# scverse/scanpy

Hardware: AMD Instinct MI355X
Metric: cells/sec through pca+neighbors+leiden, 1M x 2k CSR (higher is better)
Workload: dtype bf16x3

## Files before the change

### scanpy_amd/csrc/leiden.hip

```cpp
#include "common.h"
#include "scan.h"

#include <algorithm>
#include <cmath>
#include <cstdlib>
#include <ctime>
#include <type_traits>

namespace scamd {

enum LdStat : int {
  ST_ITERATIONS = 0, ST_LAUNCHES, ST_ROUND_TRIPS, ST_POLISH_FULL_SWEEPS, ST_POLISH_ROUNDS, ST_POLISH_MOVES,
  ST_POLISH_SKIPPED_PROVEN, ST_LEVELS_FIRST_ITER, ST_LM_SWEEPS, ST_LM_SWEEP_MB, ST_POLISH_SPLITS, ST_ENDED_BY_ITER_CAP,
  ST_POLISH_ROUND_CAP, ST_ITER_CAP, ST_UNUSED_14, ST_DEVICE_FILLS, ST_LEVELS_REUSED, ST_QUIET_REUSE_ITERS,
  ST_OVERFLOW_VERTICES, ST_HUB_VERTICES, LD_NSTATS
};
static_assert(LD_NSTATS == 20 && ST_UNUSED_14 == 14, "the slot numbers are part of the C ABI (scamd_leiden_last_stats)");
struct LdStatName {
  int slot;
  const char* key;
};
static const LdStatName LD_STAT_NAMES[] = {
    {ST_ITERATIONS, "iterations"},
    {ST_LAUNCHES, "launches"},
    {ST_ROUND_TRIPS, "host_round_trips"},
    {ST_POLISH_FULL_SWEEPS, "polish_full_sweeps"},
    {ST_POLISH_ROUNDS, "polish_rounds"},
    {ST_POLISH_MOVES, "polish_moves"},
    {ST_POLISH_SKIPPED_PROVEN, "polish_skipped_proven"},
    {ST_LEVELS_FIRST_ITER, "levels_first_iteration"},
    {ST_LM_SWEEPS, "lm_sweeps"},
    {ST_LM_SWEEP_MB, "lm_sweep_algorithmic_MB"},
    {ST_POLISH_SPLITS, "polish_splits"},
    {ST_ENDED_BY_ITER_CAP, "ended_by_iteration_cap"},
    {ST_POLISH_ROUND_CAP, "polish_ended_by_round_cap"},
    {ST_ITER_CAP, "iteration_cap"},
    {ST_DEVICE_FILLS, "device_fills"},
    {ST_LEVELS_REUSED, "levels_reused"},
    {ST_QUIET_REUSE_ITERS, "quiet_reuse_iterations"},
    {ST_OVERFLOW_VERTICES, "overflow_pass_vertices"},
    {ST_HUB_VERTICES, "hub_pass_vertices"},
};
constexpr int G16_SLOTS = 128;
constexpr int G16_MAX = G16_SLOTS * 3 / 4;
static thread_local int g_ld_stats[LD_NSTATS] = {0};
static thread_local double g_ld_sweep_bytes = 0.0;
#undef SCAMD_LAUNCH_CHECK
#define SCAMD_LAUNCH_CHECK()                \
  do {                                      \
    ++g_ld_stats[ST_LAUNCHES];              \
    SCAMD_HIP_CHECK(hipGetLastError());     \
  } while (0)
#define LD_FETCH(dst, src, bytes, stream)                                          \
  do {                                                                             \
    const int rc_fetch_ = host_readback().fetch((dst), (src), (bytes), (stream)); \
    if (rc_fetch_ != SCAMD_OK) return rc_fetch_;                                   \
  } while (0)
#define LD_SYNC(stream)                                       \
  do {                                                        \
    ++g_ld_stats[ST_ROUND_TRIPS];                             \
    const int rc_sync_ = host_readback().sync(stream);        \
    if (rc_sync_ != SCAMD_OK) return rc_sync_;                \
  } while (0)

constexpr double WSCALE = 4294967296.0;
constexpr int MAX_LM_SWEEPS = 96;
constexpr int LM_DIR_AFTER = 32;
constexpr int MAX_CLASSES = 32;
constexpr int DEF_CLASSES = 8;
constexpr int CTR_STRIDE = 16;
constexpr int CTR_JOINED = 0, CTR_N_MID = 8, CTR_N_BLK = 9, CTR_N_GIANT = 10;
constexpr int PH_PER_PHASE = 8;
constexpr int PH_MOVED = 0, PH_BLOCKED = 1;
constexpr int PH_CC_CHANGED = 2, PH_CC_COMPONENTS = 3, PH_CC_COMMUNITIES = 4;
constexpr int PH_AGG_PART_SLOTS = 2, PH_AGG_PARTS = 3, PH_AGG_MID = 4, PH_AGG_BIG = 5, PH_AGG_SPLIT = 6;
constexpr int PHASE_ERR = 7;
constexpr int PH_MAX_DEG = 8;
constexpr int PH_SMALL_INFO = 12, SM_INFO_LEVELS = 0, SM_INFO_MOVES = 1, SM_INFO_MERGES = 2, SM_INFO_NODES = 3;
constexpr int CTR_AREA = MAX_CLASSES + CTR_STRIDE * MAX_CLASSES;
constexpr int MAX_LEVELS = 64;
constexpr int MAX_OUTER_ITERS = 32;

__host__ __device__ __forceinline__ unsigned int hash32(unsigned int x) {
  x ^= x >> 16;
  x *= 0x7feb352dU;
  x ^= x >> 15;
  x *= 0x846ca68bU;
  x ^= x >> 16;
  return x;
}
__device__ __forceinline__ unsigned int prio(int c, unsigned int seed) { return hash32((unsigned int)c ^ seed); }

__device__ __forceinline__ long long readlane_i64(long long v, int l) {
  int lo = __builtin_amdgcn_readlane((int)(v & 0xffffffffll), l);
  int hi = __builtin_amdgcn_readlane((int)(v >> 32), l);
  return ((long long)hi << 32) | (unsigned int)lo;
}

__global__ void ld_quantize_kernel(const float* __restrict__ w, int64_t nnz, long long* __restrict__ wq) {
  int64_t e = (int64_t)blockIdx.x * blockDim.x + threadIdx.x;
  if (e < nnz) {
    double v = (double)w[e];
    wq[e] = (v > 0.0) ? (long long)llrint(v * WSCALE) : 0ll;
  }
}

__global__ void ld_strength_kernel(const int64_t* __restrict__ indptr, const long long* __restrict__ wq, int n,
                                   long long* __restrict__ k) {
  const int lane = threadIdx.x & 63;
  const int v = blockIdx.x * (blockDim.x >> 6) + (threadIdx.x >> 6);
  if (v >= n) return;
  long long s = 0;
  for (int64_t e = indptr[v] + lane; e < indptr[v + 1]; e += 64) s += wq[e];
#pragma unroll
  for (int o = 32; o > 0; o >>= 1) s += __shfl_xor(s, o);
  if (lane == 0) k[v] = s;
}

__global__ __launch_bounds__(256) void ld_sum_kernel(const long long* __restrict__ a, int n,
                                                     unsigned long long* __restrict__ total) {
  long long s = 0;
  for (int i = blockIdx.x * blockDim.x + threadIdx.x; i < n; i += gridDim.x * blockDim.x) s += a[i];
#pragma unroll
  for (int o = 32; o > 0; o >>= 1) s += __shfl_xor(s, o);
  if ((threadIdx.x & 63) == 0 && s != 0) atomicAdd(total, (unsigned long long)s);
}

__global__ __launch_bounds__(1024) void ld_degstats_kernel(const int64_t* __restrict__ indptr, int n, int* __restrict__ out) {
  __shared__ int sh;
  if (threadIdx.x == 0) sh = 0;
  __syncthreads();
  int v = blockIdx.x * blockDim.x + threadIdx.x;
  int d = (v < n) ? (int)(indptr[v + 1] - indptr[v]) : 0;
#pragma unroll
  for (int o = 32; o > 0; o >>= 1) d = max(d, __shfl_xor(d, o));
  if ((threadIdx.x & 63) == 0 && d > 0) atomicMax(&sh, d);
  __syncthreads();
  if (threadIdx.x == 0 && sh > 0) atomicMax(out, sh);
}

__global__ void ld_iota_kernel(int* __restrict__ a, int n) {
  int i = blockIdx.x * blockDim.x + threadIdx.x;
  if (i < n) a[i] = i;
}

constexpr double NODE_WEIGHT_SCALE = 65536.0;
__global__ void ld_nodeweight_quantize_kernel(const float* __restrict__ w, int n, long long* __restrict__ k, int* __restrict__ err) {
  const int v = blockIdx.x * blockDim.x + threadIdx.x;
  if (v >= n) return;
  const float x = w[v];
  if (!(x >= 0.f) || !(x <= 1.0e6f)) {
    atomicOr(err, 1);
    k[v] = 0ll;
    return;
  }
  k[v] = llrint((double)x * NODE_WEIGHT_SCALE);
// ... 1538 lines not shown
        const int64_t p = u0 + wbase + __popcll(m & ((1ull << lane) - 1ull));
        s_col[p] = key;
        s_w[p] = (long long)vals[sl];
      }
    }
    __syncthreads();
    if (threadIdx.x == 0) rowcnt[c] = sh_cnt;
    __syncthreads();
  }
}

__global__ __launch_bounds__(256) void ld_agg_compact_kernel(int nn, const int64_t* __restrict__ moff,
                                                             const int64_t* __restrict__ eoff,
                                                             const int64_t* __restrict__ indptr_new,
                                                             const int* __restrict__ s_col,
                                                             const long long* __restrict__ s_w,
                                                             int* __restrict__ out_col, long long* __restrict__ out_w,
                                                             int* __restrict__ dstat) {
  const int lane = threadIdx.x & 63;
  const int c = blockIdx.x * 4 + (threadIdx.x >> 6);
  if (blockIdx.x == 0 && threadIdx.x == 0) dstat[0] = 0;
  if (c >= nn) return;
  const int64_t u0 = eoff[moff[c]];
  const int64_t p0 = indptr_new[c];
  const int cnt = (int)(indptr_new[c + 1] - p0);
  for (int i = lane; i < cnt; i += 64) {
    out_col[p0 + i] = s_col[u0 + i];
    out_w[p0 + i] = s_w[u0 + i];
  }
}

constexpr int SMALL_N = 1024;
constexpr int SMALL_NNZ = 65536;
constexpr int SM_WAVES = 8;
constexpr int SM_THREADS = SM_WAVES * 64;

struct SmallArgs {
  const int64_t* indptr;
  const int* indices;
  const long long* wq;
  const long long* k;
  int n;
  int* ix[2];
  long long* w[2];
  int first_dst;
  int* comm;
  double gg;
  double inv_beta;
  unsigned int seed;
  int iter;
  int lm_stop_permille;
  int seq_n;
  int* info;
};

struct SmallLds {
  unsigned long long acc[SM_WAVES][SMALL_N];
  unsigned short touched[SM_WAVES][SMALL_N];
  unsigned long long Ktot[SMALL_N];
  long long kk[SMALL_N];
  int ip[SMALL_N + 1];
  int comm[SMALL_N];
  int csize[SMALL_N];
  unsigned short order[SMALL_N];
  unsigned short tail_of[SMALL_N];
  unsigned char flag[SMALL_N];
  int ref[SMALL_N];
  int refsize[SMALL_N];
  union {
    struct {
      unsigned long long Kref[SMALL_N];
      unsigned long long Eref[SMALL_N];
      long long a_in[SMALL_N];
      int stamp[SMALL_N];
    } rf;
    struct {
      int cid[SMALL_N];
      int members[SMALL_N];
      int moff[SMALL_N + 1];
      int rep[SMALL_N];
      int rowptr[SMALL_N + 1];
    } ag;
  } u;
  int tcnt[SM_WAVES];
  int dec[SM_WAVES];
  int rset[SM_WAVES];
  int scan_w[SM_WAVES];
  int s_n_act, s_moved, s_merged, s_nn;
};
static_assert(sizeof(SmallLds) <= 160 * 1024, "SmallLds must fit the 160 KB of LDS");

__device__ __forceinline__ int small_scan(int* x, int n, int* scan_w) {
  const int t = threadIdx.x, lane = t & 63, wv = t >> 6;
  const int i0 = 2 * t, i1 = 2 * t + 1;
  const int a0 = i0 < n ? x[i0] : 0, a1 = i1 < n ? x[i1] : 0;
  int inc = a0 + a1;
#pragma unroll
  for (int o = 1; o < 64; o <<= 1) {
    const int y = __shfl_up(inc, o);
    if (lane >= o) inc += y;
  }
  if (lane == 63) scan_w[wv] = inc;
  __syncthreads();
  int off = 0, tot = 0;
  for (int i = 0; i < SM_WAVES; ++i) {
    const int s = scan_w[i];
    if (i < wv) off += s;
    tot += s;
  }
  const int ex = off + inc - (a0 + a1);
  if (i0 < n) x[i0] = ex;
  if (i1 < n) x[i1] = ex + a0;
  __syncthreads();
  return tot;
}

template <typename P>
__device__ __forceinline__ int small_compact(int n, P pred, unsigned short* order, int* scan_w) {
  const int t = threadIdx.x, lane = t & 63, wv = t >> 6;
  int base = 0;
  for (int v0 = 0; v0 < n; v0 += SM_THREADS) {
    const int v = v0 + t;
    const bool f = v < n && pred(v);
    const unsigned long long m = __ballot(f);
    if (lane == 0) scan_w[wv] = __popcll(m);
    __syncthreads();
    int off = 0, tot = 0;
    for (int i = 0; i < SM_WAVES; ++i) {
      const int s = scan_w[i];
      if (i < wv) off += s;
      tot += s;
    }
    if (f) order[base + off + __popcll(m & ((1ull << lane) - 1ull))] = (unsigned short)v;
    base += tot;
    __syncthreads();
  }
  return base;
}

constexpr int SMALL_SEQ_N = 16;
__global__ __launch_bounds__(SM_THREADS) void ld_small_levels_kernel(SmallArgs a) {
// ... 292 lines not shown
          for (int mi = L.u.ag.moff[c]; mi < L.u.ag.moff[c + 1]; ++mi) {
            const int v = L.u.ag.members[mi];
            for (int e = L.ip[v] + lane; e < L.ip[v + 1]; e += 64) {
              const long long w = wq[e];
              if (w != 0) {
                const int key = L.u.ag.cid[ix[e]];
                const unsigned long long old = atomicAdd(&acc[key], (unsigned long long)w);
                if (old == 0ull) touched[atomicAdd(&L.tcnt[wv], 1)] = (unsigned short)key;
              }
            }
          }
          const int tc = __hip_atomic_load(&L.tcnt[wv], __ATOMIC_RELAXED, __HIP_MEMORY_SCOPE_WORKGROUP);
          long long ksum = 0;
          const int p0 = pass ? L.u.ag.rowptr[c] : 0;
          for (int i = lane; i < tc; i += 64) {
            const int col = touched[i];
            const unsigned long long s = acc[col];
            acc[col] = 0ull;
            if (pass) {
              nix[p0 + i] = col;
              nw[p0 + i] = (long long)s;
              ksum += (long long)s;
            }
          }
          if (pass) {
#pragma unroll
            for (int o = 32; o > 0; o >>= 1) ksum += __shfl_xor(ksum, o);
            if (lane == 0) L.kk[c] = ksum;
          } else if (lane == 0) {
            L.u.ag.rep[c] = tc;
          }
        }
      }
      __syncthreads();
      if (pass == 0) {
        for (int c = t; c < nn; c += SM_THREADS) L.u.ag.rowptr[c] = L.u.ag.rep[c];
        __syncthreads();
        const int nnz_new = small_scan(L.u.ag.rowptr, nn, L.scan_w);
        if (t == 0) L.u.ag.rowptr[nn] = nnz_new;
        __syncthreads();
      }
    }
    for (int c = t; c <= nn; c += SM_THREADS) L.ip[c] = L.u.ag.rowptr[c];
    for (int c = t; c < nn; c += SM_THREADS) L.comm[c] = L.csize[c];
    __threadfence();
    __syncthreads();
    ix = nix;
    wq = nw;
    dst ^= 1;
    n = nn;
  }
  __syncthreads();
  for (int i = t; i < n_in; i += SM_THREADS) a.comm[i] = L.comm[L.tail_of[i]];
  if (t == 0) {
    a.info[SM_INFO_LEVELS] = levels;
    a.info[SM_INFO_MOVES] = tot_moves;
    a.info[SM_INFO_MERGES] = tot_merges;
    a.info[SM_INFO_NODES] = n;
  }
}

template <int G>
__global__ __launch_bounds__(256) void ld_internal_kernel(int n, const int64_t* __restrict__ indptr,
                                                          const int* __restrict__ indices,
                                                          const long long* __restrict__ wq, const int* __restrict__ comm,
                                                          unsigned long long* __restrict__ internal) {
  const int lane = threadIdx.x & 63, sub = threadIdx.x % G;
  long long s = 0;
  for (int v = blockIdx.x * (256 / G) + threadIdx.x / G; v < n; v += gridDim.x * (256 / G)) {
    const int a = comm[v];
    const int64_t beg = indptr[v], end = indptr[v + 1];
    for (int64_t e = beg + sub; e < end; e += 4 * G) {
      int u[4], cu[4];
      long long we[4];
#pragma unroll
      for (int t = 0; t < 4; ++t) {
        const int64_t ee = e + t * G;
        u[t] = ee < end ? indices[ee] : v;
        we[t] = ee < end ? wq[ee] : 0ll;
      }
#pragma unroll
      for (int t = 0; t < 4; ++t) cu[t] = comm[u[t]];
#pragma unroll
      for (int t = 0; t < 4; ++t)
        if (cu[t] == a) s += we[t];
    }
  }
#pragma unroll
  for (int o = 32; o > 0; o >>= 1) s += __shfl_xor(s, o);
  __shared__ long long sh_s[4];
  if (lane == 0) sh_s[threadIdx.x >> 6] = s;
  __syncthreads();
  if (threadIdx.x == 0) {
    const long long tot = sh_s[0] + sh_s[1] + sh_s[2] + sh_s[3];
    if (tot != 0) atomicAdd(internal, (unsigned long long)tot);
  }
}

constexpr int SUMSQ_BLOCKS = 256;
__device__ __forceinline__ double block_sum_1024(double s, double* sh) {
  sh[threadIdx.x] = s;
  __syncthreads();
  for (int o = 512; o > 0; o >>= 1) {
    if ((int)threadIdx.x < o) sh[threadIdx.x] += sh[threadIdx.x + o];
    __syncthreads();
  }
  return sh[0];
// ... 158 lines not shown
  b->scan_tmp = ws.take<int64_t>((size_t)scan_num_blocks(n) + 2);
  b->cid = ws.take<int>(N);
  b->rep = ws.take<int>(N);
  b->comm_tmp = ws.take<int>(N);
  b->node_of = ws.take<int>(N);
  b->memb = ws.take<int>(N);
  b->memb_work = ws.take<int>(N);
  b->agg_col = ws.take<int>(E);
  b->agg_w = ws.take<long long>(E);
  b->mcount = ws.take<int>(N);
  b->moff = ws.take<int64_t>(N + 1);
  b->eoff = ws.take<int64_t>(N + 1);
  b->members = ws.take<int>(N);
  b->mdeg = ws.take<int>(N);
  b->mid_list = ws.take<int>(N);
  b->big_list = ws.take<int>(N);
  {
    const size_t slots = 3 * E / (size_t)agg_split_chunk() + 16;
    b->pmoff = ws.take<int64_t>(slots);
    b->part_list = ws.take<int>(slots);
    b->part_cnt = ws.take<int>(slots);
  }
  b->rowcnt = ws.take<int>(N);
  b->cursor = ws.take<int>(N);
  b->counters = ws.take<int>(16);
  b->rcounters = ws.take<int>(2 * CTR_AREA);
  b->total = ws.take<unsigned long long>(4);
  b->dscratch = ws.take<double>(4 + SUMSQ_BLOCKS);
  b->ckeys = ws.take<unsigned long long>(N);
  b->cids = ws.take<int>(N);
  b->newlabel = ws.take<int>(N);
  b->minmember = ws.take<int>(N);
}

#define GRID1(n) dim3((unsigned)ceil_div((n), 256)), dim3(256)
#define GRIDW(n) dim3((unsigned)ceil_div((n), 4)), dim3(256)
#define GRIDK(n) dim3((unsigned)ceil_div((n), 1024)), dim3(1024)
constexpr int HUB_GRID = 512;
constexpr int AGG_MID_GRID = 768;
constexpr int LM_STOP_PERMILLE = 20;
constexpr int LM_STOP_PERMILLE_BIG = 40;
constexpr size_t HUB_LDS = (size_t)BHUB_SLOTS * 12;

struct Hierarchy {
  int depth = 0;
  int end_level = -1;
  int end_kind = 0;
};
struct IterHierarchy {
  int built = 0;
  int end_level = -1, end_kind = 0;
  bool quiet = false;
  int small_moves = 0;
  Hierarchy accepted() const { return Hierarchy{std::max(built, 0), end_level, end_kind}; }
};

struct LeidenCtx {
  HostReadbackScope readback_scope;
  hipStream_t s;
  LeidenBuffers b;
  double gamma;
  double m2;
  bool cpm = false;
  const float* node_weights = nullptr;
  double nw_scale = 1.0;
  double gscale() const { return cpm ? gamma * WSCALE / (nw_scale * nw_scale) : gamma / m2; }
  double inv_beta = 0.0;
  int iter = 0;
  unsigned int seed;
  int l0_moves = -1;
  int n_levels = 0;
  bool debug = false;
  bool debug_sync = false;
  bool small_levels = true;
  bool polish = true;
  bool reuse = true;
  int force_lanes = 0;
  int iter_cap = MAX_OUTER_ITERS;
  int max_iters = 0;
  int agg_wave_max = WH_MAX_DEG;
  int agg_mid_max = AGG_MID_MAX;
  int agg_pass_keys = AGG_BIG_PASS;
  int agg_wave_work = 2048;
  int agg_mid_work = 65536;
  int hub_try_probes = HUB_TRY_PROBES;
  int64_t agg_split_chunk = 0, agg_split_work = 0;
  int agg_rows_mid = 0, agg_rows_big = 0, agg_rows_split = 0;
  size_t cap_e = 0, cap_p = 0, cap_c = 0;
  StoredLevel lv[MAX_LEVELS + 1];
  Hierarchy kept;
  IterHierarchy it;
};

static void read_knobs(LeidenCtx& cx) {
  cx.debug = env_is("SCAMD_LEIDEN_DEBUG", '1') || env_is("SCAMD_LEIDEN_DEBUG", '2');
  cx.debug_sync = env_is("SCAMD_LEIDEN_DEBUG", '2');
  cx.small_levels = !env_is("SCAMD_LEIDEN_SMALL", '0');
  cx.polish = !env_is("SCAMD_LEIDEN_POLISH", '0');
  cx.reuse = !env_is("SCAMD_LEIDEN_REUSE", '0');
  bool quad_set = false;
  const int quad = env_int("SCAMD_LEIDEN_QUAD", 0, &quad_set);
  cx.force_lanes = !quad_set ? 0 : (quad == 1 ? 16 : (quad == 2 ? 32 : 64));
  const int cap = env_int("SCAMD_LEIDEN_ITER_CAP", 0);
  cx.iter_cap = cap > 0 ? cap : MAX_OUTER_ITERS;
  cx.max_iters = env_int("SCAMD_LEIDEN_MAX_ITERS", 0);
  cx.agg_wave_max = std::min(env_int("SCAMD_LEIDEN_AGG_WAVE_MAX", WH_MAX_DEG), (int)WH_MAX_DEG);
  cx.agg_mid_max = std::min(env_int("SCAMD_LEIDEN_AGG_MID_MAX", AGG_MID_MAX), (int)AGG_MID_MAX);
  cx.agg_pass_keys = std::max(16, std::min(env_int("SCAMD_LEIDEN_AGG_PASS_KEYS", AGG_BIG_PASS), (int)AGG_BIG_PASS));
  cx.agg_wave_work = std::max(1, env_int("SCAMD_LEIDEN_AGG_WAVE_WORK", 2048));
  cx.agg_mid_work = std::max(1, env_int("SCAMD_LEIDEN_AGG_MID_WORK", 65536));
  cx.hub_try_probes = std::max(0, env_int("SCAMD_LEIDEN_HUB_TRY_PROBES", HUB_TRY_PROBES));
  cx.agg_split_chunk = agg_split_chunk();
  cx.agg_split_work = agg_split_work();
}

#define LD_DBG_SYNC(cx, ...)                                  \
  do {                                                        \
    if ((cx).debug_sync) {                                    \
      (void)hipStreamSynchronize((cx).s);                     \
      fprintf(stderr, "[leiden] done: " __VA_ARGS__);         \
      fputc('\n', stderr);                                    \
      fflush(stderr);                                         \
    }                                                         \
  } while (0)

struct Filler {
  FillArgs a;
  unsigned long long max_words = 0;
  Filler() { a.n = 0; }
  Filler& add(void* p, size_t bytes, unsigned int pat = 0u) {
    if (bytes == 0) return *this;
    a.p[a.n] = static_cast<unsigned int*>(p);
    a.words[a.n] = bytes / 4;
    a.pat[a.n] = pat;
    max_words = std::max<unsigned long long>(max_words, a.words[a.n]);
    ++a.n;
    return *this;
  }
};
static int run_fill(LeidenCtx& cx, const Filler& f) {
  if (f.a.n == 0) return SCAMD_OK;
  const unsigned grid = (unsigned)std::min<unsigned long long>(2048ull, std::max<unsigned long long>(1ull, (f.max_words / 4 + 255) / 256));
  hipLaunchKernelGGL(ld_fill_kernel, dim3(grid), dim3(256), 0, cx.s, f.a);
  SCAMD_LAUNCH_CHECK();
  ++g_ld_stats[ST_DEVICE_FILLS];
  return SCAMD_OK;
}

static int read_counters(LeidenCtx& cx, int* h, int cnt) {
  LD_FETCH(h, cx.b.counters, sizeof(int) * cnt, cx.s);
  LD_SYNC(cx.s);
  return SCAMD_OK;
}

template <bool WITH_32, typename F>
static void with_lanes(int lanes, F&& f) {
  if (lanes == 16) return f(std::integral_constant<int, 16>());
  if constexpr (WITH_32) {
    if (lanes == 32) return f(std::integral_constant<int, 32>());
  }
  return f(std::integral_constant<int, 64>());
}
static int blocks_for(int lanes, int cnt) { return ceil_div(cnt, 256 / lanes); }

static int compute_totals(LeidenCtx& cx, const LevelGraph& g, const int* comm, Filler extra = Filler()) {
  extra.add(cx.b.Ktot, sizeof(unsigned long long) * g.n).add(cx.b.csize, sizeof(int) * g.n);
  const int rcf = run_fill(cx, extra);
  if (rcf != SCAMD_OK) return rcf;
  hipLaunchKernelGGL(ld_totals_kernel, dim3((unsigned)std::min(REDUCE_GRID, ceil_div(g.n, 1024))), dim3(1024), 0, cx.s, comm, g.k, g.n, cx.b.Ktot, cx.b.csize,
                     cx.b.total + 1);
  SCAMD_LAUNCH_CHECK();
  return SCAMD_OK;
}

static int quality(LeidenCtx& cx, const LevelGraph& g, const int* comm, double* q) {
  constexpr int qgrid = 2048;
  with_lanes<false>(g.nnz <= (int64_t)48 * g.n ? 16 : 64, [&](auto G) {
    constexpr int L = decltype(G)::value;
    hipLaunchKernelGGL(ld_internal_kernel<L>, dim3((unsigned)std::min(qgrid, blocks_for(L, g.n))), dim3(256), 0, cx.s, g.n,
                       g.indptr, g.indices, g.wq, comm, cx.b.total + 1);
  });
  SCAMD_LAUNCH_CHECK();
  hipLaunchKernelGGL(ld_sumsq_kernel, dim3(SUMSQ_BLOCKS), dim3(1024), 0, cx.s, g.n, cx.b.Ktot, cx.cpm ? cx.nw_scale : cx.m2, cx.b.dscratch + 4);
  SCAMD_LAUNCH_CHECK();
  hipLaunchKernelGGL(ld_sumsq_final_kernel, dim3(1), dim3(1024), 0, cx.s, cx.b.dscratch + 4, cx.b.dscratch);
  SCAMD_LAUNCH_CHECK();
  unsigned long long internal = 0;
  double sumsq = 0;
  LD_FETCH(&internal, cx.b.total + 1, sizeof(internal), cx.s);
  LD_FETCH(&sumsq, cx.b.dscratch, sizeof(double), cx.s);
  LD_SYNC(cx.s);
  *q = cx.cpm ? ((double)(long long)internal - cx.gamma * WSCALE * sumsq) / cx.m2
              : (double)(long long)internal / cx.m2 - cx.gamma * sumsq;
  return SCAMD_OK;
}

static int evaluate(LeidenCtx& cx, const LevelGraph& g, const int* comm, double* q) {
  const int rc = compute_totals(cx, g, comm);
  return rc != SCAMD_OK ? rc : quality(cx, g, comm, q);
}

static_assert(WH_SLOTS / 2 * 3 / 4 == 192 && WH_MAX_DEG == 384,
              "the table ladders of the decide kernels (rows <= 96 / 192 / 384) are written out in their nslots expressions");
static int level_lanes(const LeidenCtx& cx, const LevelGraph& g) {
  if (cx.force_lanes) return cx.force_lanes;
  if (g.n <= 0) return 64;
  const int64_t avg = g.nnz / g.n;
  return avg <= 40 ? 16 : (avg <= 110 ? 32 : 64);
}
static int refine_lanes(const LeidenCtx& cx, const LevelGraph& g) { return level_lanes(cx, g) == 16 ? 16 : 64; }
static int lanes_thr_mid(int lanes) { return lanes == 16 ? (int)G16_MAX : (lanes == 32 ? (int)(WH_SLOTS / 2 * 3 / 4) : -1); }

static int giant_stride(const LevelGraph& g) { return (int)(g.nnz / (BLK_MAX_DEG + 1)) + 1; }
static TierDst tier_dst(LeidenCtx& cx, const LevelGraph& g, int lanes) {
  return TierDst{g.indptr, cx.b.tier_lists, cx.b.giant_lists, giant_stride(g), lanes_thr_mid(lanes)};
}

struct RequeueHead {
  int n_act;
  const int* list;
  const int* decision;
};
static int main_grid_cap(const MoveArgs&) { return 1 << 30; }
static int main_grid_cap(const ProposeArgs&) { return 32768; }
static void launch_fused_tiers(LeidenCtx& cx, const LevelGraph& g, int lanes, unsigned grid, const RequeueHead* rq, int nb_rq, const MoveArgs& a) {
  with_lanes<true>(lanes, [&](auto G) {
    constexpr int L = decltype(G)::value;
    if (rq)
      hipLaunchKernelGGL(ld_requeue_move_kernel<L>, dim3(grid), dim3(256), 0, cx.s, nb_rq, rq->n_act, rq->list, rq->decision, g.indptr,
                         g.indices, (const int*)cx.b.comm, cx.b.flag, a);
    else
      hipLaunchKernelGGL(ld_move_kernel<L>, dim3(grid), dim3(256), 0, cx.s, a);
  });
}
static void launch_fused_tiers(LeidenCtx& cx, const LevelGraph&, int lanes, unsigned grid, const RequeueHead*, int, const ProposeArgs& a) {
  with_lanes<false>(lanes, [&](auto G) {
    hipLaunchKernelGGL(ld_refine_propose_kernel<decltype(G)::value>, dim3(grid), dim3(256), 0, cx.s, a);
  });
}
static void launch_giant_tier(LeidenCtx& cx, unsigned grid, const MoveArgs& a, HubTry ht) {
  hipLaunchKernelGGL(ld_move_hub_kernel, dim3(grid), dim3(HUB_THREADS), HUB_LDS, cx.s, a, ht);
}
static void launch_giant_tier(LeidenCtx& cx, unsigned grid, const ProposeArgs& a, HubTry ht) {
  hipLaunchKernelGGL(ld_refine_propose_hub_kernel, dim3(grid), dim3(HUB_THREADS), HUB_LDS, cx.s, a, ht);
}
template <typename Args>
static int decide_tiers(LeidenCtx& cx, const char* what, const LevelGraph& g, int cls, int lanes, const RequeueHead* rq, const int* hctr,
// ... 429 lines not shown
      hipLaunchKernelGGL(ld_nest_check_kernel, GRID1(g.n), 0, cx.s, g.n, nn, sl.cid, (const int*)b.comm, b.comm_tmp, pass, b.counters + PHASE_ERR);
      SCAMD_LAUNCH_CHECK();
    }
    int bad = 0;
    LD_FETCH(&bad, b.counters + PHASE_ERR, sizeof(int), cx.s);
    LD_SYNC(cx.s);
    SCAMD_REQUIRE(bad == 0, SCAMD_EINTERNAL, "leiden: the stored level %d is not nested in the partition it is reused for (%d)", level + 1, bad);
  }
  int rc = run_fill(cx, Filler().add(b.rep, sizeof(int) * (size_t)g.n, 0x7f7f7f7fu));
  if (rc != SCAMD_OK) return rc;
  hipLaunchKernelGGL(ld_coarse_rep_kernel, GRIDK(g.n), 0, cx.s, g.n, sl.cid, (const int*)b.comm, b.rep);
  SCAMD_LAUNCH_CHECK();
  hipLaunchKernelGGL(ld_coarse_comm_kernel, GRID1(g.n), 0, cx.s, g.n, sl.cid, (const int*)b.comm, (const int*)b.rep, b.comm_tmp, nn, b.cursor, b.counters);
  SCAMD_LAUNCH_CHECK();
  hipLaunchKernelGGL(ld_remap_kernel, GRID1(n_orig), 0, cx.s, n_orig, sl.cid, b.node_of);
  SCAMD_LAUNCH_CHECK();
  std::swap(b.comm, b.comm_tmp);
  *out = sl.g;
  ++g_ld_stats[ST_LEVELS_REUSED];
  return SCAMD_OK;
}

struct LevelTrace {
  LeidenCtx& cx;
  double last = 0.0;
  char level[192] = "";
  double lap() {
    if (!cx.debug) return 0.0;
    (void)hipStreamSynchronize(cx.s);
    timespec ts;
    clock_gettime(CLOCK_MONOTONIC, &ts);
    const double now = ts.tv_sec * 1e3 + ts.tv_nsec * 1e-6, ms = now - last;
    last = now;
    return ms;
  }
  void moved(int l, const LevelGraph& g, int moves) {
    if (cx.debug)
      snprintf(level, sizeof(level), "[leiden] level %d n=%d nnz=%lld maxdeg=%d: local moving %.2f ms (%d moves)", l, g.n,
               (long long)g.nnz, g.max_deg, lap(), moves);
  }
  __attribute__((format(printf, 2, 3))) void say(const char* fmt, ...) const {
    if (!cx.debug) return;
    va_list ap;
    va_start(ap, fmt);
    vfprintf(stderr, fmt, ap);
    va_end(ap);
  }
};

static int small_levels(LeidenCtx& cx, const LevelGraph& g, int level) {
  LeidenBuffers& b = cx.b;
  int* info = b.counters + PH_SMALL_INFO;
  const SmallArgs a{g.indptr, g.indices, g.wq, g.k, g.n, {b.sm_ix[0], b.sm_ix[1]}, {b.sm_w[0], b.sm_w[1]}, 0, b.comm,
                    cx.gscale(), cx.inv_beta, cx.seed, cx.iter, LM_STOP_PERMILLE, SMALL_SEQ_N, info};
  hipLaunchKernelGGL(ld_small_levels_kernel, dim3(1), dim3(SM_THREADS), sizeof(SmallLds), cx.s, a);
  SCAMD_LAUNCH_CHECK();
  if (cx.debug) {
    int h[4];
    LD_FETCH(h, info, sizeof(h), cx.s);
    LD_SYNC(cx.s);
    fprintf(stderr, "[leiden] small levels from level %d (n=%d nnz=%lld): %d levels, %d moves, %d merges -> n=%d\n", level, g.n,
            (long long)g.nnz, h[SM_INFO_LEVELS], h[SM_INFO_MOVES], h[SM_INFO_MERGES], h[SM_INFO_NODES]);
  }
  return SCAMD_OK;
}

static int leiden_iteration(LeidenCtx& cx, const LevelGraph& g0) {
  LeidenBuffers& b = cx.b;
  hipLaunchKernelGGL(ld_iter_init_kernel, GRID1(g0.n), 0, cx.s, g0.n, (const int*)b.memb, b.comm, b.node_of);
  SCAMD_LAUNCH_CHECK();
  LevelGraph g = g0;
  cx.l0_moves = -1;
  bool quiet = cx.reuse && cx.iter >= 1;
  int reused = 0;
  cx.it = IterHierarchy();
  const Hierarchy& kept = cx.kept;
  LevelTrace tr{cx};
  for (int level = 0; level < MAX_LEVELS; ++level) {
    tr.lap();
    if (cx.small_levels && g.n <= SMALL_N && g.nnz <= SMALL_NNZ) {
      const int rcs = small_levels(cx, g, level);
      if (rcs != SCAMD_OK) return rcs;
      tr.say("[leiden] small levels %.2f ms\n", tr.lap());
      cx.it.end_level = level;
      if (quiet && level >= 1 && reused == level) {
        cx.it.quiet = true;
        LD_FETCH(&cx.it.small_moves, b.counters + PH_SMALL_INFO + SM_INFO_MOVES, sizeof(int), cx.s);
      }
      break;
    }
    int moves = 0;
    int rc = local_moving(cx, g, &moves);
    if (rc != SCAMD_OK) return rc;
    if (level == 0) cx.l0_moves = moves;
    cx.n_levels = level + 1;
    tr.moved(level, g, moves);
    if (moves != 0) quiet = false;
    const bool on_store = quiet && cx.it.built == level;
    if (on_store && kept.depth >= level + 1) {
      LevelGraph gs;
      rc = reuse_level(cx, g, g0.n, level, &gs);
      if (rc != SCAMD_OK) return rc;
      cx.it.built = level + 1;
      ++reused;
      tr.say("%s, reused %.2f ms -> n=%d\n", tr.level, tr.lap(), gs.n);
      g = gs;
      continue;
    }
    if (on_store && level >= 1 && reused == level && kept.depth == level && kept.end_level == level && kept.end_kind != 0) {
      tr.say("%s, reused: the last level\n", tr.level);
      cx.it.end_level = level;
      cx.it.end_kind = kept.end_kind;
      cx.it.quiet = true;
      ++g_ld_stats[ST_LEVELS_REUSED];
      break;
    }
    int merged = 0;
    rc = refinement(cx, g, &merged);
    if (rc != SCAMD_OK) return rc;
    tr.say("%s, refinement %.2f ms (%d merged)\n", tr.level, tr.lap(), merged);
    cx.it.end_level = level;
    if (merged == 0) {
      cx.it.end_kind = 1;
      break;
    }
    LevelGraph gn;
    int n_new = 0;
    rc = aggregate(cx, g, g0.n, level, &gn, &n_new);
    if (rc != SCAMD_OK) return rc;
    tr.say("[leiden] level %d aggregate %.2f ms -> n=%d\n", level, tr.lap(), n_new);
    if (n_new == g.n) {
      cx.it.end_kind = 2;
      break;
    }
    cx.it.end_level = -1;
    g = gn;
  }
  hipLaunchKernelGGL(ld_gather_kernel, GRID1(g0.n), 0, cx.s, g0.n, b.comm, b.node_of, b.memb_work);
  SCAMD_LAUNCH_CHECK();
  return SCAMD_OK;
}

static int renumber(LeidenCtx& cx, int n, int* n_comm, int* out) {
  LeidenBuffers& b = cx.b;
  {
    const int rcf = run_fill(cx, Filler().add(b.minmember, sizeof(int) * n, 0x7f7f7f7fu).add(b.csize, sizeof(int) * n));
    if (rcf != SCAMD_OK) return rcf;
  }
  hipLaunchKernelGGL(ld_minmember_kernel, dim3((unsigned)std::min(REDUCE_GRID, ceil_div(n, 1024))), dim3(1024), 0, cx.s, n, b.memb, b.minmember, b.csize);
  SCAMD_LAUNCH_CHECK();
  hipLaunchKernelGGL(ld_flag_kernel, GRID1(n), 0, cx.s, n, b.csize, b.flag, (int*)nullptr);
  SCAMD_LAUNCH_CHECK();
  int rc = exclusive_scan_i32_i64(b.flag, n, b.newid, b.scan_tmp, cx.s);
  if (rc != SCAMD_OK) return rc;
  int64_t nc = 0;
  LD_FETCH(&nc, b.newid + n, sizeof(int64_t), cx.s);
  LD_SYNC(cx.s);
  hipLaunchKernelGGL(ld_commkeys_kernel, GRID1(n), 0, cx.s, n, b.csize, b.minmember, b.newid, b.ckeys, b.cids);
  SCAMD_LAUNCH_CHECK();
  if (nc <= 131072) {
    hipLaunchKernelGGL(ld_rank_kernel, GRID1(nc), 0, cx.s, (int)nc, b.ckeys, b.cids, b.newlabel);
  } else {
    hipLaunchKernelGGL(ld_compact_label_kernel, GRID1(nc), 0, cx.s, (int)nc, b.cids, b.newlabel);
  }
  SCAMD_LAUNCH_CHECK();
  hipLaunchKernelGGL(ld_relabel_kernel, GRID1(n), 0, cx.s, n, b.newlabel, (const int*)b.memb, out);
  SCAMD_LAUNCH_CHECK();
  *n_comm = (int)nc;
  return SCAMD_OK;
}

static int setup_level0(LeidenCtx& cx, const int64_t* indptr, const int32_t* indices, const float* weights, int64_t n,
                        int64_t nnz, LevelGraph* g0) {
  LeidenBuffers& b = cx.b;
  if (nnz > 0) {
    hipLaunchKernelGGL(ld_quantize_kernel, dim3((unsigned)ceil_div(nnz, 256)), dim3(256), 0, cx.s, weights, nnz, b.wq0);
    SCAMD_LAUNCH_CHECK();
  }
  {
    const int rcf = run_fill(cx, Filler().add(b.total, sizeof(unsigned long long) * 4).add(b.counters, sizeof(int) * 16));
    if (rcf != SCAMD_OK) return rcf;
  }
  hipLaunchKernelGGL(ld_strength_kernel, GRIDW(n), 0, cx.s, indptr, b.wq0, (int)n, b.k0);
  SCAMD_LAUNCH_CHECK();
  hipLaunchKernelGGL(ld_sum_kernel, dim3(256), dim3(256), 0, cx.s, b.k0, (int)n, b.total);
  SCAMD_LAUNCH_CHECK();
  hipLaunchKernelGGL(ld_degstats_kernel, GRIDK(n), 0, cx.s, indptr, (int)n, b.counters + PH_MAX_DEG);
  SCAMD_LAUNCH_CHECK();
  unsigned long long tot = 0;
  int max_deg = 0;
  LD_FETCH(&tot, b.total, sizeof(tot), cx.s);
  LD_FETCH(&max_deg, b.counters + PH_MAX_DEG, sizeof(int), cx.s);
  LD_SYNC(cx.s);
  cx.m2 = (double)tot;
  *g0 = LevelGraph{(int)n, max_deg, nnz, indptr, indices, b.wq0, b.k0};
  if (cx.cpm && cx.node_weights) {
    hipLaunchKernelGGL(ld_nodeweight_quantize_kernel, GRID1(n), 0, cx.s, cx.node_weights, (int)n, b.k0, b.counters + PHASE_ERR);
    SCAMD_LAUNCH_CHECK();
    int bad = 0;
    LD_FETCH(&bad, b.counters + PHASE_ERR, sizeof(int), cx.s);
    LD_SYNC(cx.s);
    SCAMD_REQUIRE(bad == 0, SCAMD_EINVAL, "leiden: node weights must lie in [0, 1e6]");
    cx.nw_scale = NODE_WEIGHT_SCALE;
  } else if (cx.cpm) {
    hipLaunchKernelGGL(ld_fill_i64_kernel, GRID1(n), 0, cx.s, b.k0, (int)n, 1ll);
    SCAMD_LAUNCH_CHECK();
  }
  return SCAMD_OK;
}

static int leiden_open(LeidenCtx& cx, const char* what, const int64_t* indptr, const int32_t* indices, const float* weights,
                       int64_t n, int64_t nnz, void* workspace, size_t workspace_bytes, scamd_stream_t stream, LevelGraph* g0) {
  SCAMD_REQUIRE(indptr && (nnz == 0 || (indices && weights)), SCAMD_EINVAL, "%s: null pointer", what);
  SCAMD_REQUIRE(n >= 1 && n < ((int64_t)1 << 31) && nnz >= 0, SCAMD_EINVAL, "%s: bad shape n=%lld nnz=%lld", what, (long long)n,
                (long long)nnz);
  read_knobs(cx);
  cx.s = stream;
  cx.cap_e = 2 * (size_t)std::max<int64_t>(nnz, 1);
  cx.cap_p = 2 * ((size_t)n + 1);
  cx.cap_c = 2 * (size_t)n;
  Workspace ws(workspace, workspace_bytes);
  leiden_carve(ws, n, nnz, &cx.b);
  SCAMD_REQUIRE(workspace && ws.ok, SCAMD_EWORKSPACE, "%s: workspace %zu < required %zu", what, workspace_bytes, ws.used());
  return setup_level0(cx, indptr, indices, weights, n, nnz, g0);
}

struct LeidenCall {
  const int64_t* indptr; const int32_t* indices; const float* weights; int64_t n, nnz;
  double resolution; int n_iterations; double beta; uint64_t seed;
  int objective;
  const float* node_weights; const int32_t* initial_membership;
  int32_t* membership; double* modularity_host; int32_t* n_communities_host;
  void* workspace; size_t workspace_bytes; scamd_stream_t stream;
};

static int accept_iteration(LeidenCtx& cx, const LevelGraph& g0, int it, double* q_best, int* verdict) {
  LeidenBuffers& b = cx.b;
  cx.iter = it;
  g_ld_stats[ST_ITERATIONS] = it + 1;
  double q = 0.0;
  int rc = leiden_iteration(cx, g0);
  if (rc == SCAMD_OK) rc = evaluate(cx, g0, b.memb_work, &q);
  if (rc != SCAMD_OK) return rc;
  if (cx.debug) fprintf(stderr, "[leiden] iteration %d: Q = %.10f (best before %.10f), level-0 moves %d\n", it, q, *q_best, cx.l0_moves);
  if (cx.it.quiet && cx.it.small_moves == 0) ++g_ld_stats[ST_QUIET_REUSE_ITERS];
  *verdict = q > *q_best + 1e-12 ? 1 : (q < *q_best - 1e-12 ? -1 : 0);
  if (*verdict > 0) {
    *q_best = q;
    std::swap(b.memb, b.memb_work);
    cx.kept = cx.it.accepted();
  }
  return SCAMD_OK;
}

static int allow_dynamic_lds() {
  const struct {
    const void* kernel;
    size_t lds;
  } dyn_lds[] = {{reinterpret_cast<const void*>(ld_move_hub_kernel), HUB_LDS},
                 {reinterpret_cast<const void*>(ld_refine_propose_hub_kernel), HUB_LDS},
                 {reinterpret_cast<const void*>(ld_agg_merge_kernel), HUB_LDS},
                 {reinterpret_cast<const void*>(ld_agg_block_kernel<BHUB_SLOTS, 1024>), HUB_LDS},
                 {reinterpret_cast<const void*>(ld_small_levels_kernel), sizeof(SmallLds)}};
  for (const auto& k : dyn_lds) SCAMD_HIP_CHECK(hipFuncSetAttribute(k.kernel, hipFuncAttributeMaxDynamicSharedMemorySize, (int)k.lds));
  return SCAMD_OK;
}

static void set_rule(LeidenCtx& cx, double resolution, double beta, uint64_t seed) {
  cx.gamma = resolution;
  cx.inv_beta = beta > 0.0 ? 1.0 / (beta * WSCALE) : 0.0;
  cx.seed = (unsigned int)(seed ^ (seed >> 32)) * 0x9E3779B1u + 0x632BE5ABu;
}

static int leiden_run(const LeidenCall& c) {
  SCAMD_REQUIRE(c.membership, SCAMD_EINVAL, "leiden: null pointer");
  SCAMD_REQUIRE(c.resolution >= 0.0, SCAMD_EINVAL, "leiden: negative resolution");
  for (int i = 0; i < LD_NSTATS; ++i) g_ld_stats[i] = 0;
  g_ld_sweep_bytes = 0.0;
  const int64_t n = c.n;
  const int n_iterations = c.n_iterations;
  LeidenCtx cx;
  set_rule(cx, c.resolution, c.beta, c.seed);
  cx.cpm = c.objective == 1;
  cx.node_weights = c.node_weights;
  LevelGraph g0;
  int rc = leiden_open(cx, "leiden", c.indptr, c.indices, c.weights, n, c.nnz, c.workspace, c.workspace_bytes, c.stream, &g0);
  if (rc != SCAMD_OK) return rc;
  if (cx.cpm) cx.small_levels = false;
  rc = allow_dynamic_lds();
  if (rc != SCAMD_OK) return rc;
  LeidenBuffers& b = cx.b;
  if (c.initial_membership) {
    hipLaunchKernelGGL(ld_copy_membership_kernel, GRID1(n), 0, cx.s, (int)n, c.initial_membership, b.memb, b.counters + PHASE_ERR);
    SCAMD_LAUNCH_CHECK();
    int bad = 0;
    LD_FETCH(&bad, b.counters + PHASE_ERR, sizeof(int), cx.s);
    LD_SYNC(cx.s);
    SCAMD_REQUIRE(bad == 0, SCAMD_EINVAL, "leiden: initial membership ids must lie in [0, n)");
  } else {
    hipLaunchKernelGGL(ld_iota_kernel, GRID1(n), 0, cx.s, b.memb, (int)n);
    SCAMD_LAUNCH_CHECK();
  }
  double q_best = 0.0;
  if (cx.m2 > 0.0) {
    rc = evaluate(cx, g0, b.memb, &q_best);
    if (rc != SCAMD_OK) return rc;
    g_ld_stats[ST_ITER_CAP] = cx.iter_cap;
    int max_iter = n_iterations < 0 ? cx.iter_cap : n_iterations;
    if (n_iterations < 0 && cx.max_iters > 0) max_iter = std::min(max_iter, cx.max_iters);
    int bad_iters = 0;
    bool best_is_clean = false;
    bool ended_by_cap = true;
    for (int it = 0; it < max_iter; ++it) {
      int verdict = 0;
      rc = accept_iteration(cx, g0, it, &q_best, &verdict);
      if (rc != SCAMD_OK) return rc;
      if (it == 0) g_ld_stats[ST_LEVELS_FIRST_ITER] = cx.n_levels;
      if (verdict > 0) {
        bad_iters = 0;
        best_is_clean = false;
      } else if (cx.l0_moves == 0) {
        best_is_clean = true;
      }
      if (n_iterations < 0 && verdict <= 0) {
        ended_by_cap = false;
        if (verdict == 0 || ++bad_iters >= 2) break;
        ended_by_cap = true;
      }
    }
    int n_iter_total = g_ld_stats[ST_ITERATIONS];
    ended_by_cap = ended_by_cap && max_iter == cx.iter_cap;
    g_ld_stats[ST_ENDED_BY_ITER_CAP] = (n_iterations < 0 && ended_by_cap) ? 1 : 0;
    for (int pr = 0; n_iterations < 0 && cx.polish && pr <= MAX_POLISH_PASSES; ++pr) {
      if (best_is_clean) {
        if (pr == 0) g_ld_stats[ST_POLISH_SKIPPED_PROVEN] = 1;
        break;
      }
      PolishPass ps;
      rc = polish_level0(cx, g0, &ps);
      if (rc != SCAMD_OK) return rc;
      g_ld_stats[ST_POLISH_FULL_SWEEPS] += ps.full_sweeps;
      g_ld_stats[ST_POLISH_ROUNDS] += ps.rounds;
      g_ld_stats[ST_POLISH_MOVES] += ps.moves;
      g_ld_stats[ST_POLISH_SPLITS] += ps.splits;
      if (ps.moves == 0) break;
      cx.kept.depth = 0;
      double q = 0.0;
      rc = evaluate(cx, g0, b.memb, &q);
      if (rc != SCAMD_OK) return rc;
      if (cx.debug)
        fprintf(stderr, "[leiden] polish %d: %d full sweeps, %d rounds, %d moves: Q %.10f -> %.10f\n", pr, ps.full_sweeps, ps.rounds,
                ps.moves, q_best, q);
      SCAMD_REQUIRE(q >= q_best - 1e-12, SCAMD_EINTERNAL, "leiden: the monotone polish lowered the quality (%.12f -> %.12f)", q_best, q);
      q_best = q;
      if (pr == MAX_POLISH_PASSES || ended_by_cap) break;
      int verdict = 0;
      rc = accept_iteration(cx, g0, n_iter_total++, &q_best, &verdict);
      if (rc != SCAMD_OK) return rc;
// ... 212 lines not shown
```

Baseline: 23.09 million.

## Compute Leiden quality from coarse-level sums instead of level-0 graph walks

The per-iteration modularity evaluation now uses the top (coarsest) aggregated graph, or, when the iteration ended inside the single-block small-levels kernel, community totals and internal weight accumulated in LDS by that kernel. This avoids a full walk over the level-0 edge list each iteration. The initial quality for singleton membership is taken from the self-loop sum gathered while quantizing weights. Weight quantization and strength computation are fused into one kernel. The cost is extra work in the small kernel and a dependence on the coarse-level sums matching the level-0 quality exactly.

```diff
diff --git a/scanpy_amd/csrc/leiden.hip b/scanpy_amd/csrc/leiden.hip
--- a/scanpy_amd/csrc/leiden.hip
+++ b/scanpy_amd/csrc/leiden.hip
@@ -12,10 +12,10 @@
 enum LdStat : int {
   ST_ITERATIONS = 0, ST_LAUNCHES, ST_ROUND_TRIPS, ST_POLISH_FULL_SWEEPS, ST_POLISH_ROUNDS, ST_POLISH_MOVES,
   ST_POLISH_SKIPPED_PROVEN, ST_LEVELS_FIRST_ITER, ST_LM_SWEEPS, ST_LM_SWEEP_MB, ST_POLISH_SPLITS, ST_ENDED_BY_ITER_CAP,
-  ST_POLISH_ROUND_CAP, ST_ITER_CAP, ST_UNUSED_14, ST_DEVICE_FILLS, ST_LEVELS_REUSED, ST_QUIET_REUSE_ITERS,
+  ST_POLISH_ROUND_CAP, ST_ITER_CAP, ST_L0_QUALITY_WALKS, ST_DEVICE_FILLS, ST_LEVELS_REUSED, ST_QUIET_REUSE_ITERS,
   ST_OVERFLOW_VERTICES, ST_HUB_VERTICES, LD_NSTATS
 };
-static_assert(LD_NSTATS == 20 && ST_UNUSED_14 == 14, "the slot numbers are part of the C ABI (scamd_leiden_last_stats)");
+static_assert(LD_NSTATS == 20 && ST_L0_QUALITY_WALKS == 14, "the slot numbers are part of the C ABI (scamd_leiden_last_stats)");
 struct LdStatName {
   int slot;
   const char* key;
@@ -97,11 +97,33 @@
   return ((long long)hi << 32) | (unsigned int)lo;
 }
 
-__global__ void ld_quantize_kernel(const float* __restrict__ w, int64_t nnz, long long* __restrict__ wq) {
-  int64_t e = (int64_t)blockIdx.x * blockDim.x + threadIdx.x;
-  if (e < nnz) {
-    double v = (double)w[e];
-    wq[e] = (v > 0.0) ? (long long)llrint(v * WSCALE) : 0ll;
+__global__ __launch_bounds__(256) void ld_level0_setup_kernel(const int64_t* __restrict__ indptr, const int* __restrict__ indices,
+                                                              const float* __restrict__ w, int n, long long* __restrict__ wq,
+                                                              long long* __restrict__ k, unsigned long long* __restrict__ diag) {
+  const int lane = threadIdx.x & 63, sub = threadIdx.x & 15;
+  const int v = blockIdx.x * 16 + (threadIdx.x >> 4);
+  long long s = 0, d = 0;
+  if (v < n) {
+    const int64_t end = indptr[v + 1];
+    for (int64_t e = indptr[v] + sub; e < end; e += 16) {
+      const double x = (double)w[e];
+      const long long q = (x > 0.0) ? (long long)llrint(x * WSCALE) : 0ll;
+      wq[e] = q;
+      s += q;
+      if (indices[e] == v) d += q;
+    }
+  }
+#pragma unroll
+  for (int o = 8; o > 0; o >>= 1) s += __shfl_xor(s, o);
+  if (v < n && sub == 0) k[v] = s;
+#pragma unroll
+  for (int o = 32; o > 0; o >>= 1) d += __shfl_xor(d, o);
+  __shared__ long long sh_d[4];
+  if (lane == 0) sh_d[threadIdx.x >> 6] = d;
+  __syncthreads();
+  if (threadIdx.x == 0) {
+    const long long tot = sh_d[0] + sh_d[1] + sh_d[2] + sh_d[3];
+    if (tot != 0) atomicAdd(diag, (unsigned long long)tot);
   }
 }
 
@@ -1746,6 +1768,8 @@
   int lm_stop_permille;
   int seq_n;
   int* info;
+  unsigned long long* totals;
+  unsigned long long* internal;
 };
 
 struct SmallLds {
@@ -1781,6 +1805,7 @@
   int rset[SM_WAVES];
   int scan_w[SM_WAVES];
   int s_n_act, s_moved, s_merged, s_nn;
+  unsigned long long s_internal;
 };
 static_assert(sizeof(SmallLds) <= 160 * 1024, "SmallLds must fit the 160 KB of LDS");
 
@@ -2179,7 +2204,26 @@
   }
   __syncthreads();
   for (int i = t; i < n_in; i += SM_THREADS) a.comm[i] = L.comm[L.tail_of[i]];
+  for (int c = t; c < n_in; c += SM_THREADS) L.Ktot[c] = 0ull;
+  if (t == 0) L.s_internal = 0ull;
+  __syncthreads();
+  for (int v = t; v < n; v += SM_THREADS) atomicAdd(&L.Ktot[L.comm[v]], (unsigned long long)L.kk[v]);
+  for (int v0 = 0; v0 < n; v0 += SM_WAVES) {
+    const int v = v0 + wv;
+    if (v < n) {
+      const int ca = L.comm[v];
+      long long s = 0;
+      for (int e = L.ip[v] + lane; e < L.ip[v + 1]; e += 64)
+        if (L.comm[ix[e]] == ca) s += wq[e];
+#pragma unroll
+      for (int o = 32; o > 0; o >>= 1) s += __shfl_xor(s, o);
+      if (lane == 0 && s != 0) atomicAdd(&L.s_internal, (unsigned long long)s);
+    }
+  }
+  __syncthreads();
+  for (int c = t; c < n_in; c += SM_THREADS) a.totals[c] = L.Ktot[c];
   if (t == 0) {
+    a.internal[0] = L.s_internal;
     a.info[SM_INFO_LEVELS] = levels;
     a.info[SM_INFO_MOVES] = tot_moves;
     a.info[SM_INFO_MERGES] = tot_merges;
@@ -2444,6 +2488,8 @@
   int end_level = -1, end_kind = 0;
   bool quiet = false;
   int small_moves = 0;
+  LevelGraph top{};
+  bool in_small = false;
   Hierarchy accepted() const { return Hierarchy{std::max(built, 0), end_level, end_kind}; }
 };
 
@@ -2460,6 +2506,7 @@
   double inv_beta = 0.0;
   int iter = 0;
   unsigned int seed;
+  unsigned long long diag0 = 0;
   int l0_moves = -1;
   int n_levels = 0;
   bool debug = false;
@@ -2565,7 +2612,23 @@
   return SCAMD_OK;
 }
 
+static int quality_from_sums(LeidenCtx& cx, int n, const unsigned long long* totals, const unsigned long long* internal_host, double* q) {
+  hipLaunchKernelGGL(ld_sumsq_kernel, dim3(SUMSQ_BLOCKS), dim3(1024), 0, cx.s, n, totals, cx.cpm ? cx.nw_scale : cx.m2, cx.b.dscratch + 4);
+  SCAMD_LAUNCH_CHECK();
+  hipLaunchKernelGGL(ld_sumsq_final_kernel, dim3(1), dim3(1024), 0, cx.s, cx.b.dscratch + 4, cx.b.dscratch);
+  SCAMD_LAUNCH_CHECK();
+  unsigned long long internal = internal_host ? *internal_host : 0ull;
+  double sumsq = 0;
+  if (!internal_host) LD_FETCH(&internal, cx.b.total + 1, sizeof(internal), cx.s);
+  LD_FETCH(&sumsq, cx.b.dscratch, sizeof(double), cx.s);
+  LD_SYNC(cx.s);
+  *q = cx.cpm ? ((double)(long long)internal - cx.gamma * WSCALE * sumsq) / cx.m2
+              : (double)(long long)internal / cx.m2 - cx.gamma * sumsq;
+  return SCAMD_OK;
+}
+
 static int quality(LeidenCtx& cx, const LevelGraph& g, const int* comm, double* q) {
+  if (g.wq == cx.b.wq0) ++g_ld_stats[ST_L0_QUALITY_WALKS];
   constexpr int qgrid = 2048;
   with_lanes<false>(g.nnz <= (int64_t)48 * g.n ? 16 : 64, [&](auto G) {
     constexpr int L = decltype(G)::value;
@@ -2573,18 +2636,7 @@
                        g.indptr, g.indices, g.wq, comm, cx.b.total + 1);
   });
   SCAMD_LAUNCH_CHECK();
-  hipLaunchKernelGGL(ld_sumsq_kernel, dim3(SUMSQ_BLOCKS), dim3(1024), 0, cx.s, g.n, cx.b.Ktot, cx.cpm ? cx.nw_scale : cx.m2, cx.b.dscratch + 4);
-  SCAMD_LAUNCH_CHECK();
-  hipLaunchKernelGGL(ld_sumsq_final_kernel, dim3(1), dim3(1024), 0, cx.s, cx.b.dscratch + 4, cx.b.dscratch);
-  SCAMD_LAUNCH_CHECK();
-  unsigned long long internal = 0;
-  double sumsq = 0;
-  LD_FETCH(&internal, cx.b.total + 1, sizeof(internal), cx.s);
-  LD_FETCH(&sumsq, cx.b.dscratch, sizeof(double), cx.s);
-  LD_SYNC(cx.s);
-  *q = cx.cpm ? ((double)(long long)internal - cx.gamma * WSCALE * sumsq) / cx.m2
-              : (double)(long long)internal / cx.m2 - cx.gamma * sumsq;
-  return SCAMD_OK;
+  return quality_from_sums(cx, g.n, cx.b.Ktot, nullptr, q);
 }
 
 static int evaluate(LeidenCtx& cx, const LevelGraph& g, const int* comm, double* q) {
@@ -3120,7 +3172,7 @@
   LeidenBuffers& b = cx.b;
   int* info = b.counters + PH_SMALL_INFO;
   const SmallArgs a{g.indptr, g.indices, g.wq, g.k, g.n, {b.sm_ix[0], b.sm_ix[1]}, {b.sm_w[0], b.sm_w[1]}, 0, b.comm,
-                    cx.gscale(), cx.inv_beta, cx.seed, cx.iter, LM_STOP_PERMILLE, SMALL_SEQ_N, info};
+                    cx.gscale(), cx.inv_beta, cx.seed, cx.iter, LM_STOP_PERMILLE, SMALL_SEQ_N, info, b.Ktot, b.total + 1};
   hipLaunchKernelGGL(ld_small_levels_kernel, dim3(1), dim3(SM_THREADS), sizeof(SmallLds), cx.s, a);
   SCAMD_LAUNCH_CHECK();
   if (cx.debug) {
@@ -3151,6 +3203,7 @@
       if (rcs != SCAMD_OK) return rcs;
       tr.say("[leiden] small levels %.2f ms\n", tr.lap());
       cx.it.end_level = level;
+      cx.it.in_small = true;
       if (quiet && level >= 1 && reused == level) {
         cx.it.quiet = true;
         LD_FETCH(&cx.it.small_moves, b.counters + PH_SMALL_INFO + SM_INFO_MOVES, sizeof(int), cx.s);
@@ -3204,9 +3257,15 @@
     cx.it.end_level = -1;
     g = gn;
   }
+  cx.it.top = g;
   hipLaunchKernelGGL(ld_gather_kernel, GRID1(g0.n), 0, cx.s, g0.n, b.comm, b.node_of, b.memb_work);
   SCAMD_LAUNCH_CHECK();
   return SCAMD_OK;
+}
+
+static int iteration_quality(LeidenCtx& cx, double* q) {
+  if (cx.it.in_small) return quality_from_sums(cx, cx.it.top.n, cx.b.Ktot, nullptr, q);
+  return evaluate(cx, cx.it.top, cx.b.comm, q);
 }
 
 static int renumber(LeidenCtx& cx, int n, int* n_comm, int* out) {
@@ -3241,15 +3300,12 @@
 static int setup_level0(LeidenCtx& cx, const int64_t* indptr, const int32_t* indices, const float* weights, int64_t n,
                         int64_t nnz, LevelGraph* g0) {
   LeidenBuffers& b = cx.b;
-  if (nnz > 0) {
-    hipLaunchKernelGGL(ld_quantize_kernel, dim3((unsigned)ceil_div(nnz, 256)), dim3(256), 0, cx.s, weights, nnz, b.wq0);
-    SCAMD_LAUNCH_CHECK();
-  }
   {
     const int rcf = run_fill(cx, Filler().add(b.total, sizeof(unsigned long long) * 4).add(b.counters, sizeof(int) * 16));
     if (rcf != SCAMD_OK) return rcf;
   }
-  hipLaunchKernelGGL(ld_strength_kernel, GRIDW(n), 0, cx.s, indptr, b.wq0, (int)n, b.k0);
+  hipLaunchKernelGGL(ld_level0_setup_kernel, dim3((unsigned)ceil_div(n, 16)), dim3(256), 0, cx.s, indptr, indices, weights, (int)n,
+                     b.wq0, b.k0, b.total + 2);
   SCAMD_LAUNCH_CHECK();
   hipLaunchKernelGGL(ld_sum_kernel, dim3(256), dim3(256), 0, cx.s, b.k0, (int)n, b.total);
   SCAMD_LAUNCH_CHECK();
@@ -3259,6 +3315,7 @@
   int max_deg = 0;
   LD_FETCH(&tot, b.total, sizeof(tot), cx.s);
   LD_FETCH(&max_deg, b.counters + PH_MAX_DEG, sizeof(int), cx.s);
+  LD_FETCH(&cx.diag0, b.total + 2, sizeof(cx.diag0), cx.s);
   LD_SYNC(cx.s);
   cx.m2 = (double)tot;
   *g0 = LevelGraph{(int)n, max_deg, nnz, indptr, indices, b.wq0, b.k0};
@@ -3308,7 +3365,7 @@
   g_ld_stats[ST_ITERATIONS] = it + 1;
   double q = 0.0;
   int rc = leiden_iteration(cx, g0);
-  if (rc == SCAMD_OK) rc = evaluate(cx, g0, b.memb_work, &q);
+  if (rc == SCAMD_OK) rc = iteration_quality(cx, &q);
   if (rc != SCAMD_OK) return rc;
   if (cx.debug) fprintf(stderr, "[leiden] iteration %d: Q = %.10f (best before %.10f), level-0 moves %d\n", it, q, *q_best, cx.l0_moves);
   if (cx.it.quiet && cx.it.small_moves == 0) ++g_ld_stats[ST_QUIET_REUSE_ITERS];
@@ -3371,7 +3428,8 @@
   }
   double q_best = 0.0;
   if (cx.m2 > 0.0) {
-    rc = evaluate(cx, g0, b.memb, &q_best);
+    rc = c.initial_membership ? evaluate(cx, g0, b.memb, &q_best)
+                              : quality_from_sums(cx, g0.n, reinterpret_cast<const unsigned long long*>(g0.k), &cx.diag0, &q_best);
     if (rc != SCAMD_OK) return rc;
     g_ld_stats[ST_ITER_CAP] = cx.iter_cap;
     int max_iter = n_iterations < 0 ? cx.iter_cap : n_iterations;
```

Result: faster. 23.59 million (median of 6 runs) (+2.2%).
